# abajcsy/legged_games_gym

Hardware: AMD Instinct MI355X
Metric: env-steps/sec (whole node), ANYmal-C flat 4096 envs/GPU (higher is better)
Workload: dtype f32; 1 GPU; anymal_c_flat, 4096 envs/GPU, plane, actuator-net torques, self-collision ON (asset.self_collisions = 0), random-init policy [48, 128, 64, 32, 12] rollout (act = mu + sigma*eps), fixed command (0.5,0,0), obs noise + friction/mass randomisation + pushes on; envs_per_gpu=4096, decimation=4, parallelism=env-sharded x1, state_finite=True, policy=MFMA actor inside k_step (v_mfma_f32_16x16x4_f32, 4 waves)

## Files before the change

### legged_games_gym_amd/csrc/lg_kernels.hip

```cpp
#include <hip/hip_runtime.h>
#include <math.h>
#include <stdio.h>
#include <string.h>
#include <new>

#define LG_POLICY_BLOCKS_ONLY
#include "lg_host.h"

using namespace lg;

#define LG_BLOCK 64
#define LG_JS 40
#define LG_PASSES 2
#define LG_STEP_WAVES 4

struct AnymalTraits {
    static constexpr int K = 4, L = 3, NREP = 4, NPT = 5;
    static constexpr int pt_joint(int i) { return i < 2 ? 1 : 2; }
    static constexpr int pt_rep(int i) { return i < 2 ? 1 : (i < 4 ? 2 : 3); }
    static constexpr int FOOT_REP = 3;
    static constexpr int NCAP = 3, NGRP = 2;
    static constexpr int cap_p0(int c) { return 2 * c; }
    static constexpr int cap_p1(int c) { return c < 2 ? 2 * c + 1 : 4; }
    static constexpr int cap_grp(int c) { return c == 0 ? 0 : 1; }
// ... 1372 lines not shown
}

LG_DEV void redraw_reset_command(const KArgs &A, float x0, float x1, int e, int64_t step, float *obs_row) {
    const lg_params &P = A.P; const lg_buffers &B = A.B;
    float u[4], cmd[4];
#pragma unroll
    for (int i = 0; i < 4; i++) cmd[i] = B.commands[(size_t)e * 4 + i];
    rand4(P.seed, e, step, RNG_CMD_RESET, 0, u);
    resample_commands_x(P, x0, x1, u, cmd);
#pragma unroll
    for (int i = 0; i < 4; i++) B.commands[(size_t)e * 4 + i] = cmd[i];
    const float c = P.clip_observations;
    obs_row[9] = fminf(fmaxf(cmd[0] * P.obs_scale_lin_vel, -c), c); obs_row[10] = fminf(fmaxf(cmd[1] * P.obs_scale_lin_vel, -c), c);
    obs_row[11] = fminf(fmaxf(cmd[2] * P.obs_scale_ang_vel, -c), c);
}
LG_DEV void curriculum_apply(const KArgs &A, int t, int nt, int64_t step, float cnt, const uint8_t *resets, float *obs) {
    const lg_params &P = A.P;
    if (!(cnt > 0.0f) || P.cmd_curriculum_slot < 0) return;
    double *xr = A.B.cmd_range;
    const double mean_sum = (double)A.B.episode_means[P.cmd_curriculum_slot] * P.cmd_episode_length_s;
    const double lo0 = xr[0], hi0 = xr[1];
    if (!(mean_sum / P.cmd_max_episode_length > 0.8 * P.cmd_tracking_scale_dt)) return;
    const double lo = fmin(fmax(lo0 - 0.5, -P.cmd_max_curriculum), 0.0), hi = fmin(fmax(hi0 + 0.5, 0.0), P.cmd_max_curriculum);
    if (lo == lo0 && hi == hi0) return;
    __syncthreads();
    if (t == 0) { xr[0] = lo; xr[1] = hi; }
    const float x0 = (float)lo, x1 = (float)hi;
    for (int e = t; e < P.num_envs; e += nt)
        if (resets[e]) redraw_reset_command(A, x0, x1, e, step, obs + (size_t)e * P.num_obs);
}

template <bool OFF, int L = 3, bool HF = false> struct StepSharedT {
    float pose[LG_BLOCK][5];
    float hsum[LG_STEP_WAVES][LG_BLOCK];
    float root_z[LG_BLOCK];
    int   rst[LG_BLOCK];
    float r_t[LG_NUM_REWARD_TERMS][LG_BLOCK];
    float4 fk[OFF ? L : 1][4][LG_BLOCK];
    float4 bt[OFF ? L : 1][BtQuads<HF>::N][LG_BLOCK];
    int    fk_ready;
};

struct EpisodeSums {
    float sum[LG_NUM_REWARD_TERMS] = {};
    LG_DEV void load(const KArgs &A, int e) {
#pragma unroll
        for (int t = 0; t < LG_NUM_REWARD_TERMS; t++) {
            const int slot = A.P.reward_slot[t];
            sum[t] = slot >= 0 ? A.B.episode_sums[(size_t)slot * A.P.num_envs + e] : 0.0f;
        }
    }
    template <int K, class SH> LG_DEV void update(const KArgs &A, int e, int lane, SH &sh, bool keep, float *accum) {
        const lg_params &P = A.P;
        const bool reset = keep && sh.rst[lane] != 0;
        if (keep) {
#pragma unroll
            for (int t = 0; t < LG_NUM_REWARD_TERMS; t++) {
                const int slot = P.reward_slot[t];
                if (slot >= 0) {
                    sum[t] += sh.r_t[t][lane];
                    A.B.episode_sums[(size_t)slot * P.num_envs + e] = reset ? 0.0f : sum[t];
                }
            }
        }
        const unsigned long long finished = __ballot(reset);
        if (finished == 0) return;
#pragma unroll
        for (int t = 0; t < LG_NUM_REWARD_TERMS; t++) sh.r_t[t][lane] = reset ? sum[t] : 0.0f;
        __builtin_amdgcn_fence(__ATOMIC_RELEASE, "wavefront");
        __builtin_amdgcn_wave_barrier();
        if (lane < LG_NUM_REWARD_TERMS) {
            int slot = -1;
#pragma unroll
            for (int t = 0; t < LG_NUM_REWARD_TERMS; t++) slot = lane == t ? P.reward_slot[t] : slot;
            float tot = 0.0f;
            for (int i = 0; i < LG_BLOCK; i += K) tot += sh.r_t[lane][i];
            if (slot >= 0) atomicAdd(accum + slot, tot);
        } else if (lane == LG_NUM_REWARD_TERMS) atomicAdd(accum + P.num_reward_slots, (float)__popcll(finished));
    }
};

template <class T, bool NET, bool HF, int NW, bool SC = false> struct HelperWave {
    static constexpr bool OFF = NW >= 2;
    static LG_DEV void run(const KArgs &A, int wave, int lane, int e, int k, int d0, bool live, int64_t step, const float *tab,
                           float2 (*lds_x)[LG_BLOCK], float (*lds_tau)[LG_BLOCK], StepSharedT<OFF, T::L, HF> &sh, SelfLds<T> *sc = nullptr,
                           const float *lds_tab = nullptr, ResetRand<T> *reset_rand = nullptr, int *s_last = nullptr, float4 (*hnoise)[LG_BLOCK] = nullptr,
                           int sub0 = 0 , float *roll_accum = nullptr ,
                           bool tick_step = false ) {
        const lg_buffers &B = A.B;
        const lg_params &P = A.P;
        const int j = wave - 1;
        bool missed = false;
        LstmSplit st;
        float (*part[4])[4] = {st.h0, st.c0, st.h1, st.c1};
        float *row[4] = {nullptr, nullptr, nullptr, nullptr};
        LstmLane LW;
        if (NET) {
            const size_t plane = (size_t)P.num_envs * (T::K * T::L);
            LW = lstm_load(A.weights, lane);
            row[0] = B.sea_hidden_state + (size_t)(d0 + j) * 8; row[1] = B.sea_cell_state + (size_t)(d0 + j) * 8;
            row[2] = B.sea_hidden_state + (plane + d0 + j) * 8; row[3] = B.sea_cell_state + (plane + d0 + j) * 8;
#pragma unroll
            for (int a = 0; a < 4; a++) {
                float4 lo = reinterpret_cast<const float4 *>(row[a])[0], hi = reinterpret_cast<const float4 *>(row[a])[1];
                float u[8] = {lo.x, lo.y, lo.z, lo.w, hi.x, hi.y, hi.z, hi.w};
                lstm_split(u, part[a][0], part[a][1]);
            }
        }
        if (NET || OFF) {
            for (int it = 0; it < P.decimation; it++) {
                __syncthreads();
                float tau_j = 0.0f;
                if (NET) {
                    const float2 x = lds_x[j][lane];
                    tau_j = actuator_step_mfma(LW, x.x, x.y, st);
                    lds_tau[j][lane] = tau_j;
                }
                if (OFF) {
                    volatile int *flag = &sh.fk_ready;
                    int spin = 0;
                    for (; *flag < sub0 + it + 1 && spin < A.spin_limit; spin++) __builtin_amdgcn_s_sleep(1);
                    missed |= spin >= A.spin_limit;
#pragma unroll 1
                    for (int b = j; b < T::L; b += NW - 1) {
                        const float4 f0 = sh.fk[b][0][lane], f1 = sh.fk[b][1][lane], f2 = sh.fk[b][2][lane], f3 = sh.fk[b][3][lane];
                        M3 R; R.m[0] = f0.x; R.m[1] = f0.y; R.m[2] = f0.z; R.m[3] = f0.w; R.m[4] = f1.x; R.m[5] = f1.y; R.m[6] = f1.z; R.m[7] = f1.w; R.m[8] = f2.x;
                        const float *tb = tab + b * LG_JS;
                        float Il[6];
#pragma unroll
                        for (int i = 0; i < 6; i++) Il[i] = tb[J_INERTIA + i];
                        typename RigidOf<HF>::type I0; S6 p0;
                        body_terms(v3(P.gravity[0], P.gravity[1], P.gravity[2]), tb[J_MASS], v3(tb[J_COM], tb[J_COM + 1], tb[J_COM + 2]), Il, R,
                                   v3(f2.y, f2.z, f2.w), v3(f3.x, f3.y, f3.z), I0, p0);
                        bt_store(sh.bt[b], lane, I0, p0);
                    }
                }
                __syncthreads();
                if constexpr (SC && NW == LG_STEP_WAVES) {
                    self_detect<T>(A, lds_tab, lane, wave, *sc);
                    if (wave == LG_STEP_WAVES - 1) self_detect<T>(A, lds_tab, lane, 0, *sc);
                    asm volatile("s_waitcnt lgkmcnt(0)" ::: "memory");
                    if (lane == 0 && A.debug_skip != 2) sc->ready[wave] = sub0 + it + 1;
                }
            }
        }
        reset_rand->draw(P, e, k, step, lane, wave - 1, NW - 1);
        if (P.measure_heights && P.add_noise) {
            const int nchunk = (P.num_height_points + 3) >> 2;
#pragma unroll
            for (int b = 0; b < HeightCrew<T, NW>::NCH; b++) {
                const int c = k + b * HeightCrew<T, NW>::NV;
                if (b % (NW > 1 ? NW - 1 : 1) == wave - 1 && c < nchunk) {
                    float r[4];
                    rand4(P.seed, e, step, RNG_NOISE_H, c, r);
                    hnoise[b][lane] = make_float4(r[0], r[1], r[2], r[3]);
                }
            }
        }
        if (NET) {
#pragma unroll
            for (int a = 0; a < 4; a++) {
                float u[8];
                lstm_unsplit(part[a][0], part[a][1], u);
                if (live) {
                    reinterpret_cast<float4 *>(row[a])[0] = make_float4(u[0], u[1], u[2], u[3]);
                    reinterpret_cast<float4 *>(row[a])[1] = make_float4(u[4], u[5], u[6], u[7]);
                }
            }
        }
        __syncthreads();
        HeightCrew<T, NW> hc;
        float hs = 0.0f;
        if (P.measure_heights) hs = hc.template sample<HF>(A, e, k + T::K * wave, live, sh.pose[lane][0], sh.pose[lane][1], sh.pose[lane][2], sh.pose[lane][3], sh.pose[lane][4]);
        sh.hsum[wave][lane] = hs;
        __syncthreads();
        const bool keeper = wave == 1 && live && k == 0;
        EpisodeSums es;
        if (keeper) es.load(A, e);
        float un[HeightCrew<T, NW>::NCH][4];
        if (P.measure_heights) hc.draw_noise(P, e, k + T::K * wave, step, un);
        __syncthreads();
        if (wave == 1) {
            es.template update<T::K>(A, e, lane, sh, keeper, roll_accum ? roll_accum : accum_slot(A, step));
            if (roll_accum) {  }
            else {
            if (P.terrain_curriculum && A.B.terrain_levels) {
                int lv = keeper ? __hip_atomic_load(A.B.terrain_levels + e, __ATOMIC_RELAXED, __HIP_MEMORY_SCOPE_AGENT) : 0;
#pragma unroll
                for (int o = 32; o > 0; o >>= 1) lv += __shfl_xor(lv, o);
                if (lane == 0) __hip_atomic_store(level_parts_slot(A, step, gridDim.x) + blockIdx.x, lv, __ATOMIC_RELAXED, __HIP_MEMORY_SCOPE_AGENT);
            }
            if (tick_step) {  }
            else if (A.defer) {
                if (lane == 0 && atomicAdd(A.done_counter, 1u) == gridDim.x - 1) {
                    if (B.step_counter) B.step_counter[0] = step;
                    __hip_atomic_store(A.done_counter, 0u, __ATOMIC_RELAXED, __HIP_MEMORY_SCOPE_AGENT);
                }
            } else {
            asm volatile("s_waitcnt vmcnt(0)" ::: "memory");
            if (lane == 0) {
                const unsigned int ticket = atomicAdd(A.done_counter, 1u);
                const int last = ticket == gridDim.x - 1;
                if (last) __hip_atomic_store(A.done_counter, 0u, __ATOMIC_RELAXED, __HIP_MEMORY_SCOPE_AGENT);
                *s_last = last;
            }
            }
            }
        }
        if (P.measure_heights) hc.write_obs(A, e, k + T::K * wave, live, step, sh.root_z[lane], un);
        if (missed && lane == 0) lg_report(A.status, LG_STATUS_FRAME_HANDOVER_TIMEOUT);
        if (NET) {
            const bool reset = sh.rst[lane] != 0 && live;
            if (__ballot(reset) != 0 && reset) {
#pragma unroll
                for (int a = 0; a < 4; a++) {
                    reinterpret_cast<float4 *>(row[a])[0] = make_float4(0.0f, 0.0f, 0.0f, 0.0f);
                    reinterpret_cast<float4 *>(row[a])[1] = make_float4(0.0f, 0.0f, 0.0f, 0.0f);
                }
            }
        }
    }
};

template <bool SC, class T> struct SelfStore { char unused; LG_DEV SelfLds<T> *get() { return nullptr; } };
template <class T> struct SelfStore<true, T> { SelfLds<T> lds; LG_DEV SelfLds<T> *get() { return &lds; } };

template <class T, bool NET, bool HF, bool POL = false, int NW = LG_STEP_WAVES, bool SC = false, bool ROLL = false>
__global__ void __launch_bounds__(NW * LG_BLOCK) k_step(const KArgs A_launch) {
    const KArgs &A = A_launch;
    static_assert(!NET || (NW == LG_STEP_WAVES && 1 + T::L == NW), "one actuator wave per joint of the limb");
    static_assert(!ROLL || (POL && !HF), "the multi-step rollout kernel is the fused-actor kernel on the plane");
    static_assert(!POL || (NET && NW == LG_POLICY_WAVES && T::K * T::L <= 16), "fused policy needs the four-wave actuator-net kernel");
    constexpr int K = T::K, L = T::L, ND = K * L, NREP = T::NREP;
    const lg_params &P = A.P;
    const lg_buffers &B = A.B;
    __shared__ float lds_tab[T::K * Tab<T>::STRIDE];
    __shared__ float2 lds_x[NET ? L : 1][LG_BLOCK];
    __shared__ float lds_tau[NET ? L : 1][LG_BLOCK];
    constexpr bool OFF = NW >= 2;
    __shared__ StepSharedT<OFF, L, HF> sh;
    __shared__ SelfStore<SC, T> sc_store;
    __shared__ ResetRand<T> reset_rand;
    __shared__ float4 hnoise[NW > 1 ? HeightCrew<T, NW>::NCH : 1][LG_BLOCK];
    __shared__ int s_last;
    __shared__ float4 pol_xa[POL ? 4 : 1][64], pol_xb[POL ? 8 : 1][64], pol_xy[1][64];
    __shared__ float lds_act[POL ? 16 : 1][16];
    __shared__ float lds_obs[ROLL ? 16 : 1][48];
    __shared__ float s_tick_cnt;
    __shared__ float s_xr[2];
    __shared__ int s_roll[2];
    int roll_begin = 0;
    if (ROLL && A.P.cmd_curriculum && A.roll.sub > 0) {
        roll_begin = A.roll.cursor[0];
        if (roll_begin >= A.roll.steps) return;
    }
    LG_PROF_BEGIN();
    if (threadIdx.x == 0) sh.fk_ready = 0;
    if constexpr (SC) {
        if (threadIdx.x < LG_STEP_WAVES) sc_store.get()->ready[threadIdx.x] = 0;
        stage_base_points<T>(A, sc_store.get());
    }
    stage_limb_table<T>(A, lds_tab);

    const int N = P.num_envs;
    const int wave = threadIdx.x / LG_BLOCK, lane = threadIdx.x % LG_BLOCK;
    const int tid = blockIdx.x * LG_BLOCK + lane;
    int e = tid / K;
    const int k = tid % K;
    const bool live = e < N;
    if (!live) e = N - 1;
    const float *tab = lds_tab + k * Tab<T>::STRIDE;
    const int d0 = e * ND + k * L;
    const int64_t step0 = A.step >= 0 ? A.step : B.step_counter[0] + 1 - roll_begin;
    if (threadIdx.x == 0) {
        cmd_x_range_f32(A, s_xr);
        if (ROLL) {
            int roll_end = A.roll.steps;
            if (P.cmd_curriculum) {
                const int64_t M = P.max_episode_length, first = step0 + roll_begin;
                roll_end = min(roll_end, roll_begin + (int)((M - first % M) % M) + 1);
            }
            s_roll[0] = roll_begin; s_roll[1] = roll_end;
        }
    }
    const int e_wg = e, k_wg = k;
    auto one_step = [&](const int rt) {
    const KArgs &A = step_args<ROLL>(A_launch);
    const lg_params &P = A.P;
    const lg_buffers &B = A.B;
    const int N = P.num_envs;
    int tix = threadIdx.x;
    if constexpr (ROLL) asm volatile("" : "+v"(tix));
    const int wave = tix / LG_BLOCK, lane = tix % LG_BLOCK;
    int e = e_wg;
    const int k = ROLL ? (blockIdx.x * LG_BLOCK + lane) % K : k_wg;
    if constexpr (ROLL) { e = (blockIdx.x * LG_BLOCK + lane) / K; if (e >= N) e = N - 1; }
    const float *tab = lds_tab + k * Tab<T>::STRIDE;
    int d0 = e * ND + k * L;
    const int64_t step = step0 + rt;
    const int sub0 = ROLL ? rt * P.decimation : 0;
    float *const roll_accum = ROLL ? A.roll.extras + (size_t)rt * (LG_NUM_REWARD_TERMS + 2) : nullptr;
    float *const roll_obs_out = nullptr;

    if (POL) {
        if (ROLL) {
            PolicyArgs pa = A.pol;
            pa.obs = A.roll.obs + (size_t)rt * N * P.num_obs;
            if (rt == 0 && A.roll.obs0) {
                pa.obs = A.roll.obs0;
                const size_t row0 = (size_t)blockIdx.x * 16 * P.num_obs;
                const int n = min(16, N - (int)blockIdx.x * 16) * P.num_obs;
                for (int i = tix; i < n; i += NW * LG_BLOCK) A.roll.obs[row0 + i] = A.roll.obs0[row0 + i];
            }
            pa.actions = A.roll.actions + (size_t)rt * N * ND;
            pa.mean = A.roll.mean ? A.roll.mean + (size_t)rt * N * ND : nullptr;
            policy_forward<3, 8, 4, 2>(pa, pol_xa, pol_xb, pol_xy, blockIdx.x, wave, lane, step, lds_act, rt > s_roll[0] ? lds_obs : nullptr);
        } else policy_forward<3, 8, 4, 2>(A.pol, pol_xa, pol_xb, pol_xy, blockIdx.x, wave, lane, step, lds_act);
        __syncthreads();
    }
    if (wave > 0) {
        HelperWave<T, NET, HF, NW, SC>::run(A, wave, lane, e, k, d0, live, step, tab, lds_x, lds_tau, sh, sc_store.get(), lds_tab, &reset_rand, &s_last, hnoise, sub0, roll_accum,
                                            !ROLL && curriculum_tick_step(A, step));
    } else {
    float root[13], q[L], qd[L], act[L], tau[L];
#pragma unroll
    for (int i = 0; i < 13; i++) root[i] = B.root_states[(size_t)e * 13 + i];
#pragma unroll
    for (int j = 0; j < L; j++) {
        float2 s = reinterpret_cast<const float2 *>(B.dof_state)[d0 + j];
        q[j] = s.x; qd[j] = s.y;
        float a = POL ? lds_act[k * L + j][lane / K] : A.actions_in[d0 + j];
        act[j] = fminf(fmaxf(a, -P.clip_actions), P.clip_actions);
        tau[j] = 0.0f;
    }
    const float mu = 0.5f * ((B.friction_coeffs ? B.friction_coeffs[e] : 1.0f) + P.ground_friction);
    const float base_mass = A.base.mass + (B.base_mass_delta ? B.base_mass_delta[e] : 0.0f);
    float last_qd[L];
    if (L <= 3) {
#pragma unroll
        for (int j = 0; j < L; j++) last_qd[j] = B.last_dof_vel[d0 + j];
    }

    float Frep[NREP][3], Fbase[3];
    {
        const float *cf = B.contact_forces + ((size_t)e * (1 + K * NREP) + 1 + k * NREP) * 3;
#pragma unroll
        for (int r = 0; r < NREP; r++) { Frep[r][0] = cf[3 * r]; Frep[r][1] = cf[3 * r + 1]; Frep[r][2] = cf[3 * r + 2]; }
        const float *c0 = B.contact_forces + (size_t)e * (1 + K * NREP) * 3;
        Fbase[0] = c0[0]; Fbase[1] = c0[1]; Fbase[2] = c0[2];
    }
    if (P.decimation == 0) {
#pragma unroll
        for (int j = 0; j < L; j++) tau[j] = B.torques[d0 + j];
    }
    LG_PROF(PF_PROLOGUE);
#pragma unroll 1
    for (int it = 0; it < P.decimation; it++) {
        if (!NET) pd_torques<L>(P, tab, act, q, qd, B.last_dof_vel + d0, tau);
        if (NET || OFF) {
            if (NET) {
#pragma unroll
                for (int j = 0; j < L; j++) lds_x[j][lane] = make_float2(act[j] * P.action_scale + tab[j * LG_JS + J_Q0] - q[j], qd[j]);
            }
            __syncthreads();
            auto join = [&]() {
                __syncthreads();
                if (NET) {
#pragma unroll
                    for (int j = 0; j < L; j++) tau[j] = lds_tau[j][lane];
                }
            };
            constexpr bool LEAN = NW == LG_STEP_WAVES && L <= 3 && !HF;
            physics_substep<T, HF, decltype(join), OFF, SC, LEAN, ROLL>(A, tab, k, root, q, qd, tau, base_mass, mu, Frep, Fbase, join, sh.bt, sh.fk, &sh.fk_ready, sub0 + it + 1,
                                                                  sc_store.get(), it == P.decimation - 1, SC && NW == LG_STEP_WAVES);
        } else {
            physics_substep<T, HF, NoWait, false, SC>(A, tab, k, root, q, qd, tau, base_mass, mu, Frep, Fbase, NoWait(), nullptr, nullptr, nullptr, 0,
                                                      sc_store.get(), it == P.decimation - 1);
        }
    }

    if (L > 3) {
        asm volatile("" : "+v"(e));
        d0 = e * ND + k * L;
    }
#define U_(blk, arg) (ROLL ? (blk) : (arg))
    PostHead ph; PostRew pr; PostObs po; PostStore ps; PostStoreEnv pe;
    KargFetch<PostRew> pr_f; KargFetch<PostObs> po_f; KargFetch<PostStore> ps_f; KargFetch<PostStoreEnv> pe_f;
    if constexpr (ROLL) { KargFetch<PostHead> ph_f = karg_request(A.post.head); ph = karg_take(ph_f); }
    int64_t ep_len = U_(ph.episode_length_buf, B.episode_length_buf)[e] + 1;
    V3 blv = quat_rotate_inverse(root + 3, v3(root[7], root[8], root[9]));
    V3 bav = quat_rotate_inverse(root + 3, v3(root[10], root[11], root[12]));
    V3 pg = quat_rotate_inverse(root + 3, v3(0, 0, -1));
    float cmd[4];
#pragma unroll
    for (int i = 0; i < 4; i++) cmd[i] = U_(ph.commands, B.commands)[(size_t)e * 4 + i];
    constexpr bool EARLY_POST = L <= 3 && HF;
    float last_act[L], fat, origin[3];
    uint8_t lc;
    if (EARLY_POST) {
#pragma unroll
        for (int j = 0; j < L; j++) last_act[j] = B.last_actions[d0 + j];
        fat = B.feet_air_time[(size_t)e * K + k];
        lc = B.last_contacts[(size_t)e * K + k];
#pragma unroll
        for (int i = 0; i < 3; i++) origin[i] = B.env_origins[(size_t)e * 3 + i];
    }
    sh.pose[lane][0] = root[0]; sh.pose[lane][1] = root[1]; sh.pose[lane][2] = root[2]; sh.pose[lane][3] = root[5]; sh.pose[lane][4] = root[6];
    __syncthreads();
    if (ep_len % U_(ph.resample_interval, P.resample_interval) == 0) {
        if (NW > 1) { float u[4]; reset_rand.get(ResetRand<T>::CMD_STEP, lane, u); resample_commands_u(P, s_xr, u, cmd); }
        else resample_commands(P, s_xr, e, step, RNG_CMD_STEP, cmd);
    }
    if (U_(ph.heading_command, P.heading_command)) {
        V3 fwd = quat_apply(root + 3, v3(1, 0, 0));
        float heading = atan2f(fwd.y, fwd.x);
        cmd[2] = fminf(fmaxf(0.5f * wrap_to_pi(cmd[3] - heading), -1.0f), 1.0f);
    }
    HeightCrew<T, NW> hc;
    float hsum = 0.0f;
    if (U_(0, P.measure_heights)) hsum = hc.template sample<HF>(A, e, k, live, root[0], root[1], root[2], root[5], root[6]);
    sh.hsum[0][lane] = hsum;
    if constexpr (ROLL) pr_f = karg_request(A.post.rew);
    __syncthreads();
    if constexpr (ROLL) pr = karg_take(pr_f);
    if (NW == 4) hsum = (sh.hsum[0][lane] + sh.hsum[1][lane]) + (sh.hsum[2][lane] + sh.hsum[3][lane]);
    else if (NW == 2) hsum = sh.hsum[0][lane] + sh.hsum[1][lane];
    if (U_(ph.push_interval, P.push_interval) > 0 && step % U_(ph.push_interval, P.push_interval) == 0) {
        float u[4];
        if (NW > 1) reset_rand.get(ResetRand<T>::PUSH, lane, u);
        else rand4(P.seed, e, step, RNG_PUSH, 0, u);
        root[7] = urange(-U_(ph.max_push_vel, P.max_push_vel), U_(ph.max_push_vel, P.max_push_vel), u[0]);
        root[8] = urange(-U_(ph.max_push_vel, P.max_push_vel), U_(ph.max_push_vel, P.max_push_vel), u[1]);
    }

    const int rep0 = 1 + k * NREP;
    if (live) {
        float *cf = U_(ph.contact_forces, B.contact_forces) + ((size_t)e * (1 + K * NREP) + rep0) * 3;
#pragma unroll
        for (int r = 0; r < NREP; r++) { cf[3 * r] = Frep[r][0]; cf[3 * r + 1] = Frep[r][1]; cf[3 * r + 2] = Frep[r][2]; }
        if (k == 0) { float *c0 = U_(ph.contact_forces, B.contact_forces) + (size_t)e * (1 + K * NREP) * 3; c0[0] = Fbase[0]; c0[1] = Fbase[1]; c0[2] = Fbase[2]; }
    }
    LG_PROF(PF_POST_HEIGHTS);
    int term_local = 0;
    float coll_local = 0.0f;
#pragma unroll
    for (int r = 0; r < NREP; r++) {
        float n = sqrtf(Frep[r][0] * Frep[r][0] + Frep[r][1] * Frep[r][1] + Frep[r][2] * Frep[r][2]);
        if ((U_(ph.termination_mask, A.termination_mask) >> (rep0 + r)) & 1u) term_local |= (n > 1.0f);
        if ((U_(ph.penalised_mask, A.penalised_mask) >> (rep0 + r)) & 1u) coll_local += (n > 0.1f) ? 1.0f : 0.0f;
    }
    float nbase = sqrtf(Fbase[0] * Fbase[0] + Fbase[1] * Fbase[1] + Fbase[2] * Fbase[2]);
    int contact_term = group_or<K>(term_local);
    if (U_(ph.termination_mask, A.termination_mask) & 1u) contact_term |= (nbase > 1.0f);
    float coll = group_sum<K>(coll_local);
    if (U_(ph.penalised_mask, A.penalised_mask) & 1u) coll += (nbase > 0.1f) ? 1.0f : 0.0f;
    const bool time_out = ep_len > U_(ph.max_episode_length, P.max_episode_length);
    int bad = 0;
#pragma unroll
    for (int i = 0; i < 13; i++) bad |= !isfinite(root[i]);
#pragma unroll
    for (int j = 0; j < L; j++) bad |= !isfinite(q[j]) || !isfinite(qd[j]);
    bad = group_or<K>(bad);
    const bool reset = contact_term || time_out || bad;

    if (!EARLY_POST) {
#pragma unroll
        for (int j = 0; j < L; j++) { last_act[j] = U_(pr.last_actions, B.last_actions)[d0 + j]; if (L > 3) last_qd[j] = B.last_dof_vel[d0 + j]; }
    }
    float s_ar = 0, s_acc = 0, s_lim = 0, s_dv = 0, s_dvl = 0, s_tl = 0, s_tq = 0, s_ss = 0;
#pragma unroll
    for (int j = 0; j < L; j++) {
        const float *tj = tab + j * LG_JS;
        float da = last_act[j] - act[j]; s_ar += da * da;
        float dd = (last_qd[j] - qd[j]) / U_(pr.dt_policy, P.dt_policy); s_acc += dd * dd;
        float ol = -fminf(q[j] - tj[J_SLO], 0.0f); ol += fmaxf(q[j] - tj[J_SHI], 0.0f); s_lim += ol;
        s_dv += qd[j] * qd[j];
        s_dvl += fminf(fmaxf(fabsf(qd[j]) - tj[J_DVL] * U_(pr.soft_dof_vel_limit, P.soft_dof_vel_limit), 0.0f), 1.0f);
        s_tl += fmaxf(fabsf(tau[j]) - tj[J_TLIM] * U_(pr.soft_torque_limit, P.soft_torque_limit), 0.0f);
        s_tq += tau[j] * tau[j];
        s_ss += fabsf(q[j] - tj[J_Q0]);
    }
    s_ar = group_sum<K>(s_ar); s_acc = group_sum<K>(s_acc); s_lim = group_sum<K>(s_lim); s_dv = group_sum<K>(s_dv);
    s_dvl = group_sum<K>(s_dvl); s_tl = group_sum<K>(s_tl); s_tq = group_sum<K>(s_tq); s_ss = group_sum<K>(s_ss);
    const float *ff = Frep[T::FOOT_REP];
    const float cmd_xy = sqrtf(cmd[0] * cmd[0] + cmd[1] * cmd[1]);
    float fnorm = sqrtf(ff[0] * ff[0] + ff[1] * ff[1] + ff[2] * ff[2]);
    float fcf = group_sum<K>(fmaxf(fnorm - U_(pr.max_contact_force, P.max_contact_force), 0.0f));
    int stumble = group_or<K>(sqrtf(ff[0] * ff[0] + ff[1] * ff[1]) > 5.0f * fabsf(ff[2]) ? 1 : 0);
    float nfly = group_sum<K>(ff[2] > 0.1f ? 1.0f : 0.0f);
    float air = 0.0f;
    if (!EARLY_POST) { fat = U_(pr.feet_air_time, B.feet_air_time)[(size_t)e * K + k]; lc = U_(pr.last_contacts, B.last_contacts)[(size_t)e * K + k]; }
    if (U_(pr.reward_scale[LG_REW_FEET_AIR_TIME], P.reward_scale[LG_REW_FEET_AIR_TIME]) != 0.0f) {
        bool contact = ff[2] > 1.0f, filt = contact || lc;
        lc = (uint8_t)contact;
        bool first = (fat > 0.0f) && filt;
        fat += U_(pr.dt_policy, P.dt_policy);
        air = (fat - 0.5f) * (first ? 1.0f : 0.0f);
        fat *= filt ? 0.0f : 1.0f;
        air = group_sum<K>(air) * ((cmd_xy > 0.1f) ? 1.0f : 0.0f);
    }
    const float base_h = U_(0, P.measure_heights) ? group_sum<K>(hsum) / (float)U_(pr.num_height_points, P.num_height_points) : root[2];
    float term[LG_NUM_REWARD_TERMS];
    term[LG_REW_ACTION_RATE] = s_ar;
    term[LG_REW_ANG_VEL_XY] = bav.x * bav.x + bav.y * bav.y;
    term[LG_REW_BASE_HEIGHT] = (base_h - U_(pr.base_height_target, P.base_height_target)) * (base_h - U_(pr.base_height_target, P.base_height_target));
    term[LG_REW_COLLISION] = coll;
    term[LG_REW_DOF_ACC] = s_acc;
    term[LG_REW_DOF_POS_LIMITS] = s_lim;
    term[LG_REW_DOF_VEL] = s_dv;
    term[LG_REW_DOF_VEL_LIMITS] = s_dvl;
    term[LG_REW_FEET_AIR_TIME] = air;
    term[LG_REW_FEET_CONTACT_FORCES] = fcf;
    term[LG_REW_LIN_VEL_Z] = blv.z * blv.z;
    term[LG_REW_NO_FLY] = (nfly == 1.0f) ? 1.0f : 0.0f;
    term[LG_REW_ORIENTATION] = pg.x * pg.x + pg.y * pg.y;
    term[LG_REW_STAND_STILL] = s_ss * ((cmd_xy < 0.1f) ? 1.0f : 0.0f);
    term[LG_REW_STUMBLE] = stumble ? 1.0f : 0.0f;
    term[LG_REW_TERMINATION] = (reset && !time_out) ? 1.0f : 0.0f;
    term[LG_REW_TORQUE_LIMITS] = s_tl;
    term[LG_REW_TORQUES] = s_tq;
    {
        float ex = cmd[0] - blv.x, ey = cmd[1] - blv.y, ew = cmd[2] - bav.z;
        term[LG_REW_TRACKING_LIN_VEL] = __expf(-(ex * ex + ey * ey) / U_(pr.tracking_sigma, P.tracking_sigma));
        term[LG_REW_TRACKING_ANG_VEL] = __expf(-(ew * ew) / U_(pr.tracking_sigma, P.tracking_sigma));
    }
    LG_PROF(PF_POST_TERMS);
    float rew = 0.0f;
    const bool writer = live && k == 0;
    float r_t[LG_NUM_REWARD_TERMS];
#pragma unroll
    for (int t = 0; t < LG_NUM_REWARD_TERMS; t++) r_t[t] = U_((pr.slot_mask >> t) & 1u, P.reward_slot[t] >= 0) ? term[t] * U_(pr.reward_scale[t], P.reward_scale[t]) : 0.0f;
#pragma unroll
    for (int t = 0; t < LG_NUM_REWARD_TERMS; t++) if (t != LG_REW_TERMINATION) rew += r_t[t];
    if (U_(pr.only_positive_rewards, P.only_positive_rewards)) rew = fmaxf(rew, 0.0f);
    rew += r_t[LG_REW_TERMINATION];
#pragma unroll
    for (int t = 0; t < LG_NUM_REWARD_TERMS; t++) sh.r_t[t][lane] = r_t[t];

    LG_PROF(PF_POST_REWARD);
    if (!EARLY_POST) { const float *eo = U_(pr.env_origins, B.env_origins); origin[0] = eo[(size_t)e * 3]; origin[1] = eo[(size_t)e * 3 + 1]; origin[2] = eo[(size_t)e * 3 + 2]; }
    if (reset) {
        int level = 0; bool level_changed = false;
        reset_values<T>(A, tab, e, k, step, root, q, qd, cmd, origin, level, level_changed, s_xr, NW > 1 ? &reset_rand : nullptr, lane);
        if (writer && level_changed) {
            __hip_atomic_store(B.terrain_levels + e, level, __ATOMIC_RELAXED, __HIP_MEMORY_SCOPE_AGENT);
            B.env_origins[(size_t)e * 3] = origin[0]; B.env_origins[(size_t)e * 3 + 1] = origin[1]; B.env_origins[(size_t)e * 3 + 2] = origin[2];
        }
        fat = 0.0f; ep_len = 0;
    }

    sh.rst[lane] = reset ? 1 : 0; sh.root_z[lane] = root[2];
    if (NW > 1 && U_(pr.terrain_curriculum, P.terrain_curriculum)) asm volatile("s_waitcnt vmcnt(0)" ::: "memory");
    if constexpr (ROLL) { po_f = karg_request(A.post.obs); ps_f = karg_request(A.post.store); }
    __syncthreads();
    if constexpr (ROLL) { po = karg_take(po_f); ps = karg_take(ps_f); }
    if (NW == 1) { EpisodeSums es; const bool keep = live && k == 0; if (keep) es.load(A, e); es.template update<K>(A, e, lane, sh, keep, accum_slot(A, step)); }

    LG_PROF(PF_POST_RESET);
#ifdef LG_PROFILE
    { int nr = 0; for (int i = 0; i < LG_BLOCK; i += K) nr += sh.rst[i]; LG_PROF_NOTE(18, (unsigned long long)nr); }
#endif
    if constexpr (ROLL) write_observations<T, true>(A, e, k, live, step, root, q, qd, act, tab, blv, bav, pg, cmd, false, &reset_rand, lane,
                                                    po.roll_obs + (size_t)(rt + 1) * po.num_envs * po.num_obs, lds_obs[lane / K], &po);
    else write_observations<T>(A, e, k, live, step, root, q, qd, act, tab, blv, bav, pg, cmd, false, NW > 1 ? &reset_rand : nullptr, lane, roll_obs_out, ROLL ? lds_obs[lane / K] : nullptr);
    if (U_(0, P.measure_heights)) {
        if (NW > 1) {
            float un[HeightCrew<T, NW>::NCH][4];
#pragma unroll
            for (int b = 0; b < HeightCrew<T, NW>::NCH; b++) { const float4 w = hnoise[b][lane]; un[b][0] = w.x; un[b][1] = w.y; un[b][2] = w.z; un[b][3] = w.w; }
            hc.write_obs(A, e, k, live, step, root[2], un);
        } else hc.write_obs(A, e, k, live, step, root[2]);
    }

    LG_PROF(PF_POST_OBS);
    if constexpr (ROLL) pe_f = karg_request(A.post.store_env);
    if (live) {
#pragma unroll
        for (int j = 0; j < L; j++) {
            reinterpret_cast<float2 *>(U_(ps.dof_state, B.dof_state))[d0 + j] = make_float2(q[j], qd[j]);
            U_(ps.actions, B.actions)[d0 + j] = act[j];
            U_(ps.torques, B.torques)[d0 + j] = tau[j];
            U_(ps.last_actions, B.last_actions)[d0 + j] = act[j];
            U_(ps.last_dof_vel, B.last_dof_vel)[d0 + j] = qd[j];
        }
        U_(ps.feet_air_time, B.feet_air_time)[(size_t)e * K + k] = fat;
        U_(ps.last_contacts, B.last_contacts)[(size_t)e * K + k] = lc;
        if constexpr (ROLL) pe = karg_take(pe_f);
        if (k == 0) {
#pragma unroll
            for (int i = 0; i < 13; i++) U_(ps.root_states, B.root_states)[(size_t)e * 13 + i] = root[i];
#pragma unroll
            for (int i = 0; i < 6; i++) U_(pe.last_root_vel, B.last_root_vel)[(size_t)e * 6 + i] = root[7 + i];
#pragma unroll
            for (int i = 0; i < 4; i++) U_(pe.commands, B.commands)[(size_t)e * 4 + i] = cmd[i];
            float *const o_blv = U_(pe.base_lin_vel, B.base_lin_vel), *const o_bav = U_(pe.base_ang_vel, B.base_ang_vel), *const o_pg = U_(pe.projected_gravity, B.projected_gravity);
            o_blv[(size_t)e * 3] = blv.x; o_blv[(size_t)e * 3 + 1] = blv.y; o_blv[(size_t)e * 3 + 2] = blv.z;
            o_bav[(size_t)e * 3] = bav.x; o_bav[(size_t)e * 3 + 1] = bav.y; o_bav[(size_t)e * 3 + 2] = bav.z;
            o_pg[(size_t)e * 3] = pg.x; o_pg[(size_t)e * 3 + 1] = pg.y; o_pg[(size_t)e * 3 + 2] = pg.z;
            U_(pe.rew_buf, B.rew_buf)[e] = rew;
            U_(pe.reset_buf, B.reset_buf)[e] = (uint8_t)reset;
            U_(pe.time_out_buf, B.time_out_buf)[e] = (uint8_t)time_out;
            U_(pe.episode_length_buf, B.episode_length_buf)[e] = ep_len;
            if constexpr (ROLL) {
                pe.roll_rew[(size_t)rt * po.num_envs + e] = rew;
                pe.roll_done[(size_t)rt * po.num_envs + e] = (uint8_t)reset;
                pe.roll_time_outs[(size_t)rt * po.num_envs + e] = (uint8_t)time_out;
            }
        }
    }
#undef U_
    }
    };
    if constexpr (ROLL) {
#ifdef LG_PROFILE
        if (threadIdx.x == 0 && A.prof && blockIdx.x < LG_NPROF_BLOCKS) A.prof[LG_NPROF + LG_NPROF_BLOCKS * 40 + blockIdx.x] = wall_clock64();
#endif
        __syncthreads();
#pragma unroll 1
        for (int rt = s_roll[0]; rt < s_roll[1]; rt++) {
            one_step(rt);
            asm volatile("s_waitcnt lgkmcnt(0)\n\ts_barrier" ::: "memory");
#ifdef LG_PROFILE
            if (threadIdx.x == 0 && A.prof && blockIdx.x < LG_NPROF_BLOCKS && rt + 1 < LG_NPROF_ROLL)
                A.prof[LG_NPROF + LG_NPROF_BLOCKS * 40 + (size_t)(rt + 1) * LG_NPROF_BLOCKS + blockIdx.x] = wall_clock64();
#endif
        }
        const KArgs &A = step_args<ROLL>(A_launch);
        const lg_params &P = A.P;
        const int N = P.num_envs;
        const int roll_end = s_roll[1];
        const bool tick = P.cmd_curriculum && (step0 + roll_end - 1) % P.max_episode_length == 0;
        asm volatile("s_waitcnt vmcnt(0)" ::: "memory");
        if (tick) __threadfence();
        __syncthreads();
        if (threadIdx.x == 0) {
            const unsigned int ticket = atomicAdd(A.done_counter, 1u);
            s_last = (ticket == gridDim.x - 1);
            if (s_last) __hip_atomic_store(A.done_counter, 0u, __ATOMIC_RELAXED, __HIP_MEMORY_SCOPE_AGENT);
            if (s_last && tick) s_tick_cnt = __hip_atomic_load(A.roll.extras + (size_t)(roll_end - 1) * (LG_NUM_REWARD_TERMS + 2) + P.num_reward_slots,
                                                               __ATOMIC_RELAXED, __HIP_MEMORY_SCOPE_AGENT);
        }
        __syncthreads();
        if (s_last) {
            if (threadIdx.x < LG_BLOCK) roll_finish(A, threadIdx.x, step0, s_roll[0], roll_end);
            if (tick) {
                __threadfence();
                __syncthreads();
                curriculum_apply(A, threadIdx.x, blockDim.x, step0 + roll_end - 1, s_tick_cnt, A.roll.done + (size_t)(roll_end - 1) * N,
                                 A.roll.obs + (size_t)roll_end * N * P.num_obs);
            }
        }
        LG_PROF_END(PF_EXTRAS, A.prof);
        return;
    } else one_step(0);
    const int64_t step = step0;
    LG_PROF(PF_POST);
    if (curriculum_tick_step(A, step)) {
        __threadfence();
// ... 776 lines not shown
```

### legged_games_gym_amd/csrc/lg_policy.h

```cpp
#pragma once
#include "lg_device.h"

namespace lg {

typedef float f32x4 __attribute__((ext_vector_type(4)));

LG_DEV float elu1(float x) { return x > 0.0f ? x : (__builtin_amdgcn_exp2f(1.442695041f * x) - 1.0f); }

#define LG_POLICY_WAVES 4
template <int IN_T, int OUT_T, bool ACT>
LG_DEV void mlp_layer(const float *__restrict__ w , const float *__restrict__ b ,
                      const float4 (*xin)[64], float4 (*xout)[64], int wave, int lane) {
    constexpr int CH = IN_T > 16 ? 16 : IN_T;
#pragma unroll 1
    for (int o = wave; o < OUT_T; o += LG_POLICY_WAVES) {
        f32x4 acc;
#pragma unroll
        for (int r = 0; r < 4; r++) acc[r] = b[(o * 4 + r) * 64 + lane];
        const float *wo = w + (size_t)o * IN_T * 4 * 64 + lane;
#pragma unroll
        for (int t0 = 0; t0 < IN_T; t0 += CH) {
            float wr[CH * 4];
#pragma unroll
            for (int i = 0; i < CH * 4; i++) wr[i] = (t0 * 4 + i < IN_T * 4) ? wo[(t0 * 4 + i) * 64] : 0.0f;
            __builtin_amdgcn_sched_barrier(0);
#pragma unroll
            for (int t = 0; t < CH; t++) {
                if (t0 + t < IN_T) {
                    const float4 xv = xin[t0 + t][lane];
                    acc = __builtin_amdgcn_mfma_f32_16x16x4f32(wr[t * 4 + 0], xv.x, acc, 0, 0, 0);
                    acc = __builtin_amdgcn_mfma_f32_16x16x4f32(wr[t * 4 + 1], xv.y, acc, 0, 0, 0);
                    acc = __builtin_amdgcn_mfma_f32_16x16x4f32(wr[t * 4 + 2], xv.z, acc, 0, 0, 0);
                    acc = __builtin_amdgcn_mfma_f32_16x16x4f32(wr[t * 4 + 3], xv.w, acc, 0, 0, 0);
                }
            }
        }
        xout[o][lane] = ACT ? make_float4(elu1(acc[0]), elu1(acc[1]), elu1(acc[2]), elu1(acc[3])) : make_float4(acc[0], acc[1], acc[2], acc[3]);
    }
}

template <int IN_T> struct TileW {
    float w[IN_T * 4], b[4];
    LG_DEV void load(const float *__restrict__ wp, const float *__restrict__ bp, int o, int lane) {
#pragma unroll
        for (int i = 0; i < IN_T * 4; i++) w[i] = wp[((size_t)o * IN_T * 4 + i) * 64 + lane];
#pragma unroll
        for (int r = 0; r < 4; r++) b[r] = bp[(o * 4 + r) * 64 + lane];
    }
    template <bool ACT> LG_DEV float4 run(const float4 (*xin)[64], int lane) const {
        f32x4 acc = {b[0], b[1], b[2], b[3]};
#pragma unroll
        for (int t = 0; t < IN_T; t++) {
            const float4 xv = xin[t][lane];
            acc = __builtin_amdgcn_mfma_f32_16x16x4f32(w[t * 4 + 0], xv.x, acc, 0, 0, 0);
            acc = __builtin_amdgcn_mfma_f32_16x16x4f32(w[t * 4 + 1], xv.y, acc, 0, 0, 0);
            acc = __builtin_amdgcn_mfma_f32_16x16x4f32(w[t * 4 + 2], xv.z, acc, 0, 0, 0);
            acc = __builtin_amdgcn_mfma_f32_16x16x4f32(w[t * 4 + 3], xv.w, acc, 0, 0, 0);
        }
        return ACT ? make_float4(elu1(acc[0]), elu1(acc[1]), elu1(acc[2]), elu1(acc[3])) : make_float4(acc[0], acc[1], acc[2], acc[3]);
    }
};

struct PolicyArgs {
    const float *obs;
    const float *w[4];
    const float *b[4];
    const float *std;
    float *actions;
    float *mean;
    const int64_t *step_counter;
    int64_t step;
    uint64_t seed;
    int32_t num_envs, num_obs, num_actions, deterministic;
};

template <int D0T, int D1T, int D2T, int D3T>
LG_DEV void policy_forward(const PolicyArgs &A, float4 (*xa)[64], float4 (*xb)[64], float4 (*xy)[64], int block, int wave, int lane,
                           int64_t step, float (*lds_act)[16], const float (*lds_obs)[48] = nullptr ) {
    const int g = lane >> 4;
    int env = block * 16 + (lane & 15);
    const bool live = env < A.num_envs;
    if (!live) env = A.num_envs - 1;
    constexpr bool PRELOAD = D0T <= 4 && D1T == 2 * LG_POLICY_WAVES && D2T == LG_POLICY_WAVES && D3T == 2;
    TileW<PRELOAD ? D0T : 1> w0a, w0b;
    TileW<PRELOAD ? D1T : 1> w1;
    TileW<PRELOAD ? D2T : 1> w2;
    TileW<PRELOAD ? D3T : 1> w3;
    if constexpr (PRELOAD) {
        w0a.load(A.w[0], A.b[0], wave, lane); w0b.load(A.w[0], A.b[0], wave + LG_POLICY_WAVES, lane);
        w1.load(A.w[1], A.b[1], wave, lane);
        if (wave < D3T) w2.load(A.w[2], A.b[2], wave, lane);
        if (wave == 0) w3.load(A.w[3], A.b[3], 0, lane);
    }
    const float *o = A.obs + (size_t)env * A.num_obs;
    for (int t = wave; t < D0T; t += LG_POLICY_WAVES) {
        float v[4];
#pragma unroll
        for (int r = 0; r < 4; r++) { int k = 16 * t + 4 * g + r; v[r] = k < A.num_obs ? (lds_obs ? lds_obs[lane & 15][k] : o[k]) : 0.0f; }
        xa[t][lane] = make_float4(v[0], v[1], v[2], v[3]);
    }
    __syncthreads();
    if constexpr (PRELOAD) {
        xb[wave][lane] = w0a.template run<true>(xa, lane);
        xb[wave + LG_POLICY_WAVES][lane] = w0b.template run<true>(xa, lane);
    } else mlp_layer<D0T, D1T, true>(A.w[0], A.b[0], xa, xb, wave, lane);
    __syncthreads();
    if constexpr (PRELOAD) xa[wave][lane] = w1.template run<true>(xb, lane);
    else mlp_layer<D1T, D2T, true>(A.w[1], A.b[1], xb, xa, wave, lane);
    __syncthreads();
    if constexpr (PRELOAD) { if (wave < D3T) xb[wave][lane] = w2.template run<true>(xa, lane); }
    else mlp_layer<D2T, D3T, true>(A.w[2], A.b[2], xa, xb, wave, lane);
    if (wave == LG_POLICY_WAVES - 1) {
        float u[4];
        rand4(A.seed ^ 0x9E3779B97F4A7C15ull, env, step, 100 + g, 0, u);
        float rad0 = sqrtf(-2.0f * __logf(fmaxf(u[0], 1e-12f))), rad1 = sqrtf(-2.0f * __logf(fmaxf(u[2], 1e-12f)));
        float s0, c0, s1, c1;
        __sincosf(6.2831853f * u[1], &s0, &c0);
        __sincosf(6.2831853f * u[3], &s1, &c1);
        const float eps[4] = {rad0 * c0, rad0 * s0, rad1 * c1, rad1 * s1};
        float ns[4];
#pragma unroll
        for (int r = 0; r < 4; r++) { const int a = 4 * g + r; ns[r] = (a < A.num_actions && !A.deterministic) ? A.std[a] * eps[r] : 0.0f; }
        xy[0][lane] = make_float4(ns[0], ns[1], ns[2], ns[3]);
    }
    __syncthreads();
    if (wave != 0) return;
    const float4 nv = xy[0][lane];
    const float ns[4] = {nv.x, nv.y, nv.z, nv.w};
    if constexpr (PRELOAD) xy[0][lane] = w3.template run<false>(xb, lane);
    else mlp_layer<D3T, 1, false>(A.w[3], A.b[3], xb, xy, 0, lane);
    const float4 yv = xy[0][lane];
    const float y[4] = {yv.x, yv.y, yv.z, yv.w};
#pragma unroll
    for (int r = 0; r < 4; r++) {
        int a = 4 * g + r;
        if (a < A.num_actions) {
            float m = y[r], act = m + ns[r];
            if (lds_act) lds_act[a][lane & 15] = act;
            if (live) {
                if (A.mean) A.mean[(size_t)env * A.num_actions + a] = m;
                A.actions[(size_t)env * A.num_actions + a] = act;
            }
        }
    }
}

template <int D0T, int D1T, int D2T, int D3T>
__global__ void __launch_bounds__(64 * LG_POLICY_WAVES) k_policy_act(const PolicyArgs A) {
    constexpr int TA = D0T > D2T ? D0T : D2T, TB = D1T > D3T ? D1T : D3T;
    __shared__ float4 xa[TA][64], xb[TB][64], xy[1][64];
    const int64_t step = A.step >= 0 ? A.step : (A.step_counter ? A.step_counter[0] + 1 : 0);
    policy_forward<D0T, D1T, D2T, D3T>(A, xa, xb, xy, blockIdx.x, threadIdx.x >> 6, threadIdx.x & 63, step, nullptr);
}

typedef __bf16 bf16x8g __attribute__((ext_vector_type(8)));
typedef float f32x16p __attribute__((ext_vector_type(16)));
#define LG_PW_ENVS 32
#define LG_PW_WAVES 8
#define LG_PW_INFLIGHT 32

struct PolicyWideArgs {
    PolicyArgs base;
    const bf16x8g *wb[4];
    const float *bb[4];
};

LG_DEV void split8(const float (&v)[8], bf16x8g &hi, bf16x8g &lo) {
#pragma unroll
    for (int i = 0; i < 8; i++) { hi[i] = (__bf16)v[i]; lo[i] = (__bf16)(v[i] - (float)hi[i]); }
}

template <int KS, int TPW> struct WideStream {
    static constexpr int PF = (LG_PW_INFLIGHT / (2 * TPW) + 1) < KS + 1 ? (LG_PW_INFLIGHT / (2 * TPW) + 1) : KS + 1;
    bf16x8g wh[PF][TPW], wl[PF][TPW];
    LG_DEV void fetch(const bf16x8g *__restrict__ w, int o0, int rot, int lane, int s) {
        int sr = s + rot; sr = sr >= KS ? sr - KS : sr;
#pragma unroll
        for (int t = 0; t < TPW; t++) {
            const bf16x8g *q = w + ((size_t)((o0 + t) * KS + sr) * 2) * 64 + lane;
            wh[s % PF][t] = q[0]; wl[s % PF][t] = q[64];
        }
    }
    LG_DEV void prime(const bf16x8g *__restrict__ w, int o0, int rot, int lane) {
#pragma unroll
        for (int s = 0; s < PF - 1; s++) if (s < KS) fetch(w, o0, rot, lane, s);
    }
    LG_DEV void run(const bf16x8g *__restrict__ w, const bf16x8g (*xin)[2][64], int o0, int rot, int lane, f32x16p (&acc)[TPW]) {
#pragma unroll
        for (int t = 0; t < TPW; t++)
#pragma unroll
            for (int i = 0; i < 16; i++) acc[t][i] = 0.0f;
#pragma unroll
        for (int s = 0; s < KS; s++) {
            if (s + PF - 1 < KS) fetch(w, o0, rot, lane, s + PF - 1);
            int sr = s + rot; sr = sr >= KS ? sr - KS : sr;
            const bf16x8g bh = xin[sr][0][lane], bl = xin[sr][1][lane];
#pragma unroll
            for (int t = 0; t < TPW; t++) {
                acc[t] = __builtin_amdgcn_mfma_f32_32x32x16_bf16(wl[s % PF][t], bh, acc[t], 0, 0, 0);
                acc[t] = __builtin_amdgcn_mfma_f32_32x32x16_bf16(wh[s % PF][t], bl, acc[t], 0, 0, 0);
                acc[t] = __builtin_amdgcn_mfma_f32_32x32x16_bf16(wh[s % PF][t], bh, acc[t], 0, 0, 0);
            }
        }
    }
};

template <int TPW>
LG_DEV void wide_epilogue(const f32x16p (&acc)[TPW], const float *__restrict__ b, bf16x8g (*xout)[2][64], int o0, int lane) {
    const int h = lane >> 5;
#pragma unroll
// ... 347 lines not shown
```

Before: 78.44 million env-steps/s.

## Carry per-lane env state in LDS across rollout steps and precompute next policy noise

In the multi-step rollout kernel, commands, last actions, feet air time, origins, last contacts and episode length are loaded once into shared memory and carried across substeps instead of being re-read from global memory each step. The Gaussian action noise for the next step is also drawn early by a helper wave during the current step and read from LDS by the policy. This moves the noise math off the policy critical path. It adds LDS footprint, which may lower occupancy. It also assumes L==3 and a correct carry update on resets.

```diff
diff --git a/legged_games_gym_amd/csrc/lg_kernels.hip b/legged_games_gym_amd/csrc/lg_kernels.hip
--- a/legged_games_gym_amd/csrc/lg_kernels.hip
+++ b/legged_games_gym_amd/csrc/lg_kernels.hip
@@ -1478,11 +1478,13 @@
 
 template <class T, bool NET, bool HF, int NW, bool SC = false> struct HelperWave {
     static constexpr bool OFF = NW >= 2;
+    template <bool NEXT_NOISE = false >
     static LG_DEV void run(const KArgs &A, int wave, int lane, int e, int k, int d0, bool live, int64_t step, const float *tab,
                            float2 (*lds_x)[LG_BLOCK], float (*lds_tau)[LG_BLOCK], StepSharedT<OFF, T::L, HF> &sh, SelfLds<T> *sc = nullptr,
                            const float *lds_tab = nullptr, ResetRand<T> *reset_rand = nullptr, int *s_last = nullptr, float4 (*hnoise)[LG_BLOCK] = nullptr,
                            int sub0 = 0 , float *roll_accum = nullptr ,
-                           bool tick_step = false ) {
+                           bool tick_step = false ,
+                           float4 *pol_noise = nullptr ) {
         const lg_buffers &B = A.B;
         const lg_params &P = A.P;
         const int j = wave - 1;
@@ -1541,6 +1543,12 @@
             }
         }
         reset_rand->draw(P, e, k, step, lane, wave - 1, NW - 1);
+        if constexpr (NEXT_NOISE) if (wave == NW - 1) {
+            const int g = lane >> 4, en = min((int)blockIdx.x * 16 + (lane & 15), A.pol.num_envs - 1);
+            float sd[4];
+            policy_std(A.pol, g, sd);
+            pol_noise[lane] = policy_noise(A.pol, en, step + 1, g, sd);
+        }
         if (P.measure_heights && P.add_noise) {
             const int nchunk = (P.num_height_points + 3) >> 2;
 #pragma unroll
@@ -1642,6 +1650,10 @@
     __shared__ float4 pol_xa[POL ? 4 : 1][64], pol_xb[POL ? 8 : 1][64], pol_xy[1][64];
     __shared__ float lds_act[POL ? 16 : 1][16];
     __shared__ float lds_obs[ROLL ? 16 : 1][48];
+    __shared__ float4 pol_noise[ROLL ? 64 : 1];
+    __shared__ float4 carry_cmd[ROLL ? LG_BLOCK : 1], carry_act[ROLL ? LG_BLOCK : 1] , carry_org[ROLL ? LG_BLOCK : 1] ;
+    __shared__ int64_t carry_ep[ROLL ? LG_BLOCK : 1];
+    static_assert(!ROLL || L == 3, "carried lane records hold three dofs");
     __shared__ float s_tick_cnt;
     __shared__ float s_xr[2];
     __shared__ int s_roll[2];
@@ -1668,6 +1680,15 @@
     const float *tab = lds_tab + k * Tab<T>::STRIDE;
     const int d0 = e * ND + k * L;
     const int64_t step0 = A.step >= 0 ? A.step : B.step_counter[0] + 1 - roll_begin;
+    if constexpr (ROLL) {
+        if (wave == 0) {
+            carry_cmd[lane] = make_float4(B.commands[(size_t)e * 4], B.commands[(size_t)e * 4 + 1], B.commands[(size_t)e * 4 + 2], B.commands[(size_t)e * 4 + 3]);
+            carry_act[lane] = make_float4(B.last_actions[d0], B.last_actions[d0 + 1], B.last_actions[d0 + 2], B.feet_air_time[(size_t)e * K + k]);
+            carry_org[lane] = make_float4(B.env_origins[(size_t)e * 3], B.env_origins[(size_t)e * 3 + 1], B.env_origins[(size_t)e * 3 + 2],
+                                          __int_as_float((int)B.last_contacts[(size_t)e * K + k]));
+            carry_ep[lane] = B.episode_length_buf[e];
+        }
+    }
     if (threadIdx.x == 0) {
         cmd_x_range_f32(A, s_xr);
         if (ROLL) {
@@ -1710,13 +1731,14 @@
             }
             pa.actions = A.roll.actions + (size_t)rt * N * ND;
             pa.mean = A.roll.mean ? A.roll.mean + (size_t)rt * N * ND : nullptr;
-            policy_forward<3, 8, 4, 2>(pa, pol_xa, pol_xb, pol_xy, blockIdx.x, wave, lane, step, lds_act, rt > s_roll[0] ? lds_obs : nullptr);
+            policy_forward<3, 8, 4, 2>(pa, pol_xa, pol_xb, pol_xy, blockIdx.x, wave, lane, step, lds_act, rt > s_roll[0] ? lds_obs : nullptr,
+                                           rt > s_roll[0] ? pol_noise : nullptr);
         } else policy_forward<3, 8, 4, 2>(A.pol, pol_xa, pol_xb, pol_xy, blockIdx.x, wave, lane, step, lds_act);
         __syncthreads();
     }
     if (wave > 0) {
-        HelperWave<T, NET, HF, NW, SC>::run(A, wave, lane, e, k, d0, live, step, tab, lds_x, lds_tau, sh, sc_store.get(), lds_tab, &reset_rand, &s_last, hnoise, sub0, roll_accum,
-                                            !ROLL && curriculum_tick_step(A, step));
+        HelperWave<T, NET, HF, NW, SC>::template run<ROLL>(A, wave, lane, e, k, d0, live, step, tab, lds_x, lds_tau, sh, sc_store.get(), lds_tab, &reset_rand, &s_last, hnoise, sub0, roll_accum,
+                                            !ROLL && curriculum_tick_step(A, step), ROLL ? pol_noise : nullptr);
     } else {
     float root[13], q[L], qd[L], act[L], tau[L];
 #pragma unroll
@@ -1783,13 +1805,16 @@
     PostHead ph; PostRew pr; PostObs po; PostStore ps; PostStoreEnv pe;
     KargFetch<PostRew> pr_f; KargFetch<PostObs> po_f; KargFetch<PostStore> ps_f; KargFetch<PostStoreEnv> pe_f;
     if constexpr (ROLL) { KargFetch<PostHead> ph_f = karg_request(A.post.head); ph = karg_take(ph_f); }
-    int64_t ep_len = U_(ph.episode_length_buf, B.episode_length_buf)[e] + 1;
+    int64_t ep_len = (ROLL ? carry_ep[lane] : B.episode_length_buf[e]) + 1;
     V3 blv = quat_rotate_inverse(root + 3, v3(root[7], root[8], root[9]));
     V3 bav = quat_rotate_inverse(root + 3, v3(root[10], root[11], root[12]));
     V3 pg = quat_rotate_inverse(root + 3, v3(0, 0, -1));
     float cmd[4];
-#pragma unroll
-    for (int i = 0; i < 4; i++) cmd[i] = U_(ph.commands, B.commands)[(size_t)e * 4 + i];
+    if constexpr (ROLL) { const float4 c = carry_cmd[lane]; cmd[0] = c.x; cmd[1] = c.y; cmd[2] = c.z; cmd[3] = c.w; }
+    else {
+#pragma unroll
+        for (int i = 0; i < 4; i++) cmd[i] = B.commands[(size_t)e * 4 + i];
+    }
     constexpr bool EARLY_POST = L <= 3 && HF;
     float last_act[L], fat, origin[3];
     uint8_t lc;
@@ -1859,9 +1884,10 @@
     bad = group_or<K>(bad);
     const bool reset = contact_term || time_out || bad;
 
-    if (!EARLY_POST) {
-#pragma unroll
-        for (int j = 0; j < L; j++) { last_act[j] = U_(pr.last_actions, B.last_actions)[d0 + j]; if (L > 3) last_qd[j] = B.last_dof_vel[d0 + j]; }
+    if constexpr (ROLL) { const float4 c = carry_act[lane]; last_act[0] = c.x; last_act[1] = c.y; last_act[L - 1] = c.z; fat = c.w; }
+    else if (!EARLY_POST) {
+#pragma unroll
+        for (int j = 0; j < L; j++) { last_act[j] = B.last_actions[d0 + j]; if (L > 3) last_qd[j] = B.last_dof_vel[d0 + j]; }
     }
     float s_ar = 0, s_acc = 0, s_lim = 0, s_dv = 0, s_dvl = 0, s_tl = 0, s_tq = 0, s_ss = 0;
 #pragma unroll
@@ -1885,7 +1911,8 @@
     int stumble = group_or<K>(sqrtf(ff[0] * ff[0] + ff[1] * ff[1]) > 5.0f * fabsf(ff[2]) ? 1 : 0);
     float nfly = group_sum<K>(ff[2] > 0.1f ? 1.0f : 0.0f);
     float air = 0.0f;
-    if (!EARLY_POST) { fat = U_(pr.feet_air_time, B.feet_air_time)[(size_t)e * K + k]; lc = U_(pr.last_contacts, B.last_contacts)[(size_t)e * K + k]; }
+    if constexpr (ROLL) { const float4 c = carry_org[lane]; origin[0] = c.x; origin[1] = c.y; origin[2] = c.z; lc = (uint8_t)__float_as_int(c.w); }
+    else if (!EARLY_POST) { fat = B.feet_air_time[(size_t)e * K + k]; lc = B.last_contacts[(size_t)e * K + k]; }
     if (U_(pr.reward_scale[LG_REW_FEET_AIR_TIME], P.reward_scale[LG_REW_FEET_AIR_TIME]) != 0.0f) {
         bool contact = ff[2] > 1.0f, filt = contact || lc;
         lc = (uint8_t)contact;
@@ -1934,7 +1961,7 @@
     for (int t = 0; t < LG_NUM_REWARD_TERMS; t++) sh.r_t[t][lane] = r_t[t];
 
     LG_PROF(PF_POST_REWARD);
-    if (!EARLY_POST) { const float *eo = U_(pr.env_origins, B.env_origins); origin[0] = eo[(size_t)e * 3]; origin[1] = eo[(size_t)e * 3 + 1]; origin[2] = eo[(size_t)e * 3 + 2]; }
+    if (!ROLL && !EARLY_POST) { const float *eo = B.env_origins; origin[0] = eo[(size_t)e * 3]; origin[1] = eo[(size_t)e * 3 + 1]; origin[2] = eo[(size_t)e * 3 + 2]; }
     if (reset) {
         int level = 0; bool level_changed = false;
         reset_values<T>(A, tab, e, k, step, root, q, qd, cmd, origin, level, level_changed, s_xr, NW > 1 ? &reset_rand : nullptr, lane);
@@ -1970,6 +1997,12 @@
 
     LG_PROF(PF_POST_OBS);
     if constexpr (ROLL) pe_f = karg_request(A.post.store_env);
+    if constexpr (ROLL) {
+        carry_cmd[lane] = make_float4(cmd[0], cmd[1], cmd[2], cmd[3]);
+        carry_act[lane] = make_float4(act[0], act[1], act[L - 1], fat);
+        carry_org[lane] = make_float4(origin[0], origin[1], origin[2], __int_as_float((int)lc));
+        carry_ep[lane] = ep_len;
+    }
     if (live) {
 #pragma unroll
         for (int j = 0; j < L; j++) {
diff --git a/legged_games_gym_amd/csrc/lg_policy.h b/legged_games_gym_amd/csrc/lg_policy.h
--- a/legged_games_gym_amd/csrc/lg_policy.h
+++ b/legged_games_gym_amd/csrc/lg_policy.h
@@ -74,13 +74,33 @@
     int32_t num_envs, num_obs, num_actions, deterministic;
 };
 
+LG_DEV void policy_std(const PolicyArgs &A, int g, float (&sd)[4]) {
+#pragma unroll
+    for (int r = 0; r < 4; r++) sd[r] = A.std[min(4 * g + r, A.num_actions - 1)];
+}
+LG_DEV float4 policy_noise(const PolicyArgs &A, int env, int64_t step, int g, const float (&sd)[4]) {
+    float u[4];
+    rand4(A.seed ^ 0x9E3779B97F4A7C15ull, env, step, 100 + g, 0, u);
+    float rad0 = sqrtf(-2.0f * __logf(fmaxf(u[0], 1e-12f))), rad1 = sqrtf(-2.0f * __logf(fmaxf(u[2], 1e-12f)));
+    float s0, c0, s1, c1;
+    __sincosf(6.2831853f * u[1], &s0, &c0);
+    __sincosf(6.2831853f * u[3], &s1, &c1);
+    const float eps[4] = {rad0 * c0, rad0 * s0, rad1 * c1, rad1 * s1};
+    float ns[4];
+#pragma unroll
+    for (int r = 0; r < 4; r++) { const int a = 4 * g + r; ns[r] = (a < A.num_actions && !A.deterministic) ? sd[r] * eps[r] : 0.0f; }
+    return make_float4(ns[0], ns[1], ns[2], ns[3]);
+}
+
 template <int D0T, int D1T, int D2T, int D3T>
 LG_DEV void policy_forward(const PolicyArgs &A, float4 (*xa)[64], float4 (*xb)[64], float4 (*xy)[64], int block, int wave, int lane,
-                           int64_t step, float (*lds_act)[16], const float (*lds_obs)[48] = nullptr ) {
+                           int64_t step, float (*lds_act)[16], const float (*lds_obs)[48] = nullptr ,
+                           const float4 *noise_in = nullptr ) {
     const int g = lane >> 4;
     int env = block * 16 + (lane & 15);
     const bool live = env < A.num_envs;
     if (!live) env = A.num_envs - 1;
+    const bool draws = wave == LG_POLICY_WAVES - 1 && !noise_in;
     constexpr bool PRELOAD = D0T <= 4 && D1T == 2 * LG_POLICY_WAVES && D2T == LG_POLICY_WAVES && D3T == 2;
     TileW<PRELOAD ? D0T : 1> w0a, w0b;
     TileW<PRELOAD ? D1T : 1> w1;
@@ -92,6 +112,8 @@
         if (wave < D3T) w2.load(A.w[2], A.b[2], wave, lane);
         if (wave == 0) w3.load(A.w[3], A.b[3], 0, lane);
     }
+    float sd[4];
+    policy_std(A, g, sd);
     const float *o = A.obs + (size_t)env * A.num_obs;
     for (int t = wave; t < D0T; t += LG_POLICY_WAVES) {
         float v[4];
@@ -110,22 +132,10 @@
     __syncthreads();
     if constexpr (PRELOAD) { if (wave < D3T) xb[wave][lane] = w2.template run<true>(xa, lane); }
     else mlp_layer<D2T, D3T, true>(A.w[2], A.b[2], xa, xb, wave, lane);
-    if (wave == LG_POLICY_WAVES - 1) {
-        float u[4];
-        rand4(A.seed ^ 0x9E3779B97F4A7C15ull, env, step, 100 + g, 0, u);
-        float rad0 = sqrtf(-2.0f * __logf(fmaxf(u[0], 1e-12f))), rad1 = sqrtf(-2.0f * __logf(fmaxf(u[2], 1e-12f)));
-        float s0, c0, s1, c1;
-        __sincosf(6.2831853f * u[1], &s0, &c0);
-        __sincosf(6.2831853f * u[3], &s1, &c1);
-        const float eps[4] = {rad0 * c0, rad0 * s0, rad1 * c1, rad1 * s1};
-        float ns[4];
-#pragma unroll
-        for (int r = 0; r < 4; r++) { const int a = 4 * g + r; ns[r] = (a < A.num_actions && !A.deterministic) ? A.std[a] * eps[r] : 0.0f; }
-        xy[0][lane] = make_float4(ns[0], ns[1], ns[2], ns[3]);
-    }
+    if (draws) xy[0][lane] = policy_noise(A, env, step, g, sd);
     __syncthreads();
     if (wave != 0) return;
-    const float4 nv = xy[0][lane];
+    const float4 nv = noise_in ? noise_in[lane] : xy[0][lane];
     const float ns[4] = {nv.x, nv.y, nv.z, nv.w};
     if constexpr (PRELOAD) xy[0][lane] = w3.template run<false>(xb, lane);
     else mlp_layer<D3T, 1, false>(A.w[3], A.b[3], xb, xy, 0, lane);
```

Result: no change. 78.83 million env-steps/s (median of 6 runs) (+0.5%).
